# Sudaraka88/LDWeaver

Hardware: NVIDIA B200
Metric: weighted SNP-pair MI/sec (higher is better)
Workload: dtype int8 (tcgen05 kind::i8 with int32 accumulation of 28-bit fixed-point weights; fp32 MI epilogue, fp64 refinement of long-range links)

## Files before the change

### ldweaver_b200/csrc/mi_kernel.cuh

```cuda
#pragma once
#include "mi_types.h"
#include "umma.cuh"

namespace ldw {

constexpr int MI_EXP_WARPS = 6;
constexpr int MI_EXP_THREADS = 32 * MI_EXP_WARPS;
constexpr int MI_EPI_WARP0 = 8;
constexpr int MI_EPI_GROUPS = 4;
constexpr int MI_EPI_WARPS = 4 * MI_EPI_GROUPS;
constexpr int MI_EPI_THREADS = 32 * MI_EPI_WARPS;
constexpr int MI_THREADS = 32 * (MI_EPI_WARP0 + MI_EPI_WARPS);
#define LDW_STR2(x) #x
#define LDW_STR(x) LDW_STR2(x)
#define MI_REGS_CTRL 48
#define MI_REGS_EPI 96
static_assert(MI_EPI_WARP0 * 32 * MI_REGS_CTRL + MI_EPI_THREADS * MI_REGS_EPI <= MI_THREADS * ((65536 / MI_THREADS) & ~7), "register budget");
constexpr int MI_MAX_STAGES = 4;
constexpr uint32_t MI_ARR_BYTES = 128 * 128;
constexpr uint32_t MI_STAGE_REGION = 12 * MI_ARR_BYTES;
__host__ __device__ constexpr uint32_t mi_stage_need(int pa, int pb, int njlog2) {
  return (uint32_t)pa * MI_ARR_BYTES + 4u * (uint32_t)pb * (64u << njlog2);
}
__host__ __device__ constexpr int mi_stage_geo(int pa, int pb, int njlog2) {
  return mi_stage_need(pa, pb, njlog2) <= 3 * MI_ARR_BYTES ? 0 : mi_stage_need(pa, pb, njlog2) <= 4 * MI_ARR_BYTES ? 1 : 2;
}
__host__ __device__ constexpr int mi_geo_stages(int geo) { return 4 - geo; }
__host__ __device__ constexpr uint32_t mi_geo_bytes(int geo) { return geo == 0 ? 3 * MI_ARR_BYTES : geo == 1 ? 4 * MI_ARR_BYTES : 6 * MI_ARR_BYTES; }
constexpr uint32_t MI_JREC_BYTES = 128 * sizeof(Rec);
constexpr uint32_t MI_JDYN_BYTES = 128 * sizeof(ColDyn);
constexpr uint32_t MI_IREC_BYTES = 128 * sizeof(Rec);
constexpr uint32_t MI_IDYN_BYTES = 128 * sizeof(RowDyn);
constexpr uint32_t MI_BAR_BYTES = 512;
constexpr uint32_t MI_SMEM_BYTES = MI_STAGE_REGION + 2 * (MI_JREC_BYTES + MI_JDYN_BYTES) + MI_IREC_BYTES + MI_IDYN_BYTES + MI_BAR_BYTES + 1024;
static_assert(MI_SMEM_BYTES <= 232448, "shared memory budget (227 KB opt-in)");

__device__ __forceinline__ float lg2_fast(float x) {
  float y;
  asm("lg2.approx.ftz.f32 %0, %1;" : "=f"(y) : "f"(x));
  return y;
}
__device__ __forceinline__ uint32_t ld_volatile_u32(const uint32_t* p) {
  uint32_t v;
  asm volatile("ld.volatile.global.u32 %0, [%1];" : "=r"(v) : "l"(p));
  return v;
}

__host__ __device__ constexpr int mi_jc(int pa, int pb) {
  return (pa + 1) * (pb + 1) <= 4 ? 8 : (pa + 1) * (pb + 1) <= 9 ? 4 : (pa + 1) * (pb + 1) <= 12 ? 2 : 1;
}
__host__ __device__ constexpr int mi_njlog2(int pa, int pb) {
  return pa * pb == 1 ? 7 : pa * pb == 2 ? 6 : pa * pb <= 4 ? 5 : 4;
}

__device__ __noinline__ void lr_raise_threshold(const ScanParams& p, int lane) {
  constexpr int PER = MI_HIST_BINS / 32;
  uint32_t s = 0;
  for (int k = 0; k < PER; k++) s += ld_volatile_u32(p.hist + lane * PER + k);
  uint32_t suf = s;
#pragma unroll
  for (int o = 1; o < 32; o <<= 1) {
    uint32_t v = __shfl_down_sync(0xffffffffu, suf, o);
    if (lane + o < 32) suf += v;
  }
  unsigned m = __ballot_sync(0xffffffffu, suf >= p.kprime);
  if (m == 0) return;
  int sel = 31 - __clz(m);
  if (lane == sel) {
    uint32_t run = suf - s;
    for (int k = PER - 1; k >= 0; k--) {
      run += ld_volatile_u32(p.hist + lane * PER + k);
      if (run >= p.kprime) {
        atomicMax(p.tcand_bits, (uint32_t)(lane * PER + k) << 19);
        break;
      }
    }
  }
}

template <bool DBG>
__device__ __forceinline__ void timed_wait(uint64_t* bar, uint32_t parity, int tag, long long& acc) {
  if constexpr (DBG) {
    long long c0 = clock64();
    mbar_wait(bar, parity, tag);
    acc += clock64() - c0;
  } else {
    mbar_wait(bar, parity, tag);
  }
}

struct EpiCtx {
  int q, cg, lane, rank;
  uint32_t tflags;
// ... 267 lines not shown
  k.M = p.M;
  k.nf = p.nf; k.nt = p.nt;
  k.mul_a = 1u << p.sa; k.sb = p.sb;
  k.ragged = p.ragged != 0; k.dense = p.dense != 0;
  k.do_lr = !p.sr_only && !p.dense;
  k.has_sr = (c.tflags & TILE_HAS_SR) != 0;
  k.sr_out = p.sr_out;
  k.tcand = (k.do_lr && !p.emit_all) ? __uint_as_float(ld_volatile_u32(p.tcand_bits)) : -3.0e38f;
  uint32_t r0, r1;
  {
    const uint32_t rv = c.irec_saddr + (uint32_t)row * (uint32_t)sizeof(Rec);
    const uint4 v0 = lds128(rv), v1 = lds128(rv + (QC ? 32 : 16));
    uint4 v3 = make_uint4(0, 0, 0, 0);
    if (RA == 5) v3 = lds128(rv + 48);
    asm volatile("ld.shared.v2.u32 {%0, %1}, [%2];" : "=r"(r0), "=r"(r1) : "r"(c.idyn_saddr + (uint32_t)row * (uint32_t)sizeof(RowDyn)));
    {
      const uint32_t dep = (v0.x ^ v0.y ^ v0.z ^ v0.w ^ v1.x ^ v1.y ^ v1.z ^ v1.w ^ v3.x ^ v3.y ^ v3.z ^ r0 ^ r1);
      asm volatile("st.volatile.shared.u32 [%0], %1;" ::"r"(c.scr_saddr), "r"(dep) : "memory");
      __syncwarp();
      if (c.lane == 0) asm volatile("mbarrier.arrive.shared::cta.b64 _, [%0];" ::"r"(c.rempty_saddr) : "memory");
    }
    const uint32_t tt[5] = {v0.x, v0.y, v0.z, v0.w, v3.x}, tr[5] = {v1.x, v1.y, v1.z, v1.w, QC ? v3.z : v3.y};
    const float rf = QC ? p.rp_qc[RA - 2][RB - 2] : p.rp_plain[RA - 2][RB - 2];
#pragma unroll
    for (int a = 0; a < RA; a++) {
      k.Ti[a] = tt[a];
      k.rpad[a] = __uint_as_float(tr[a]) * rf;
    }
  }
  k.il = (int)r0;
  k.rtlq = __uint_as_float(r1) * k.qod;
// ... 47 lines not shown
  Rec* irec = reinterpret_cast<Rec*>(smem + MI_STAGE_REGION + 2 * (MI_JREC_BYTES + MI_JDYN_BYTES));
  RowDyn* idyn = reinterpret_cast<RowDyn*>(smem + MI_STAGE_REGION + 2 * (MI_JREC_BYTES + MI_JDYN_BYTES) + MI_IREC_BYTES);
  uint64_t* bars = reinterpret_cast<uint64_t*>(smem + MI_STAGE_REGION + 2 * (MI_JREC_BYTES + MI_JDYN_BYTES) + MI_IREC_BYTES + MI_IDYN_BYTES);
  uint64_t* full = bars;
  uint64_t* empty = bars + 4;
  uint64_t* ready = bars + 8;
  uint64_t* tfull = bars + 12;
  uint64_t* tempty = bars + 14;
  uint64_t* jfull = bars + 16;
  uint64_t* jempty = bars + 18;
  uint64_t* drained = bars + 20;
  uint64_t* rfull = bars + 21;
  uint64_t* rempty = bars + 22;
  uint32_t* tmem_slot = reinterpret_cast<uint32_t*>(bars + 23);
  uint32_t* thdr = reinterpret_cast<uint32_t*>(bars + 24);

  const int warp = threadIdx.x >> 5, lane = threadIdx.x & 31;
  const uint32_t rank = cluster_ctarank();
  if (warp == 0 && lane == 0) {
    tma_prefetch_desc(&tm.a);
    for (int i = 0; i < MI_MAX_STAGES; i++) {
      mbar_init(&full[i], 1); mbar_init(&empty[i], 1); mbar_init(&ready[i], 2 * MI_EXP_WARPS);
    }
    mbar_init(drained, 1);
    mbar_init(rfull, 1); mbar_init(rempty, MI_EPI_WARPS);
    for (int i = 0; i < 2; i++) {
      mbar_init(&tfull[i], 1); mbar_init(&tempty[i], 2 * MI_EPI_WARPS);
      mbar_init(&jfull[i], 1); mbar_init(&jempty[i], MI_EPI_WARPS);
    }
    fence_barrier_init();
  }
  if (warp == 2) tmem_alloc_pair(tmem_slot, 512);
  tc_fence_before();
  cluster_sync_all();
  tc_fence_after();
  const uint32_t tmem_base = *tmem_slot;
  const int tile0 = (int)(blockIdx.x >> 1), tstep = (int)(gridDim.x >> 1);

  if (warp < MI_EPI_WARP0) {
  asm volatile("setmaxnreg.dec.sync.aligned.u32 " LDW_STR(MI_REGS_CTRL) ";");
  if (warp == 0) {
    int st = 0; uint32_t phb = 0; int geo = -1; uint32_t dph = 0;
    int it = 0, rit = 0;
    long long w_jempty = 0, w_empty = 0, t_begin = DBG ? clock64() : 0;
    for (int t = tile0; t < p.n_tiles; t += tstep, it++) {
      const TileDesc td = p.tiles[t];
      const int PA = td.PA, PB = td.PB, NJ = 1 << td.njlog2, NJh = NJ >> 1;
      const int njidx = 7 - td.njlog2;
      const int g = mi_stage_geo(PA, PB, td.njlog2);
      const int nst = mi_geo_stages(g);
      const uint32_t sbytes = mi_geo_bytes(g);
      if (g != geo) {
        if (geo >= 0) { mbar_wait(drained, dph, 12); dph ^= 1; }
        geo = g; st = 0;
      }
      {
        const uint32_t stage_tx = (uint32_t)PA * MI_ARR_BYTES + (uint32_t)(PB * NJh * 128);
        const int a_row = td.a_row0 + (int)rank * 128, b_row = td.b_row0 + (int)rank * NJh;
        for (int kb = 0; kb < p.nkb; kb++) {
          timed_wait<DBG>(&empty[st], ((phb >> st) & 1) ^ 1, 11, w_empty);
          if (elect_one()) {
            uint8_t* sb = stage_base + st * sbytes;
            mbar_arrive_expect_tx(&full[st], stage_tx);
            for (int a = 0; a < PA; a++)
              tma_load_2d(sb + a * MI_ARR_BYTES, &tm.a, &full[st], kb * 128, a_row + a * td.a_pstride);
            uint8_t* sbB = sb + PA * MI_ARR_BYTES;
            for (int b = 0; b < PB; b++)
              tma_load_2d(sbB + b * NJh * 128, &tm.b[njidx], &full[st], kb * 128, b_row + b * td.b_pstride);
          }
          __syncwarp();
          phb ^= 1u << st;
          if (++st == nst) st = 0;
        }
      }
      const int jb = it & 1;
      timed_wait<DBG>(&jempty[jb], ((it >> 1) & 1) ^ 1, 10, w_jempty);
      if (elect_one()) {
        thdr[jb] = (uint32_t)PA | ((uint32_t)PB << 8) | ((uint32_t)td.njlog2 << 16) | ((uint32_t)(rank ? td.flags1 : td.flags) << 24);
        mbar_arrive_expect_tx(&jfull[jb], (uint32_t)NJ * (uint32_t)(sizeof(Rec) + sizeof(ColDyn)));
        bulk_load_1d(jrec + jb * 128, p.rec + (int64_t)(PA + 1 - 2) * p.rec_vstride + td.j_slot0, NJ * sizeof(Rec), &jfull[jb]);
        bulk_load_1d(jdyn + jb * 128, p.coldyn + td.j_dyn0, NJ * sizeof(ColDyn), &jfull[jb]);
      }
      __syncwarp();
      if (!((rank ? td.flags1 : td.flags) & TILE_NULL)) {
        timed_wait<DBG>(rempty, (uint32_t)(rit & 1) ^ 1, 13, w_jempty);
        if (elect_one()) {
          mbar_arrive_expect_tx(rfull, MI_IREC_BYTES + MI_IDYN_BYTES);
          bulk_load_1d(irec, p.rec + (int64_t)(PB + 1 - 2) * p.rec_vstride + td.i_slot0 + (int)rank * 128, MI_IREC_BYTES, rfull);
          bulk_load_1d(idyn, p.rowdyn + td.i_dyn0 + (int)rank * 128, MI_IDYN_BYTES, rfull);
        }
        __syncwarp();
        rit++;
      }
    }
    if (DBG && p.dbg && lane == 0) {
      p.dbg[blockIdx.x * 16 + 0] = (unsigned long long)(clock64() - t_begin);
      p.dbg[blockIdx.x * 16 + 1] = (unsigned long long)w_jempty;
      p.dbg[blockIdx.x * 16 + 2] = (unsigned long long)w_empty;
    }
  } else if (warp == 1) {
    if (rank == 0) {
    int st = 0; uint32_t phb = 0; int geo = -1; int as = 0; uint32_t aph = 0;
    long long w_tempty = 0, w_ready = 0, t_begin = DBG ? clock64() : 0;
    const uint32_t desc_hi = (uint32_t)(make_smem_desc_sw128(0) >> 32);
    for (int t = tile0; t < p.n_tiles; t += tstep) {
      const TileDesc td = p.tiles[t];
      const int PA = td.PA, PB = td.PB, NJ = 1 << td.njlog2;
      const int g = mi_stage_geo(PA, PB, td.njlog2);
      const int nst = mi_geo_stages(g);
      const uint32_t sbytes = mi_geo_bytes(g);
      if (g != geo) { geo = g; st = 0; }
      bool sw = false;
      if (t + tstep < p.n_tiles) {
        const TileDesc tn = p.tiles[t + tstep];
        sw = mi_stage_geo(tn.PA, tn.PB, tn.njlog2) != g;
      }
      const bool big = 2 * PA * PB * NJ > 256;
      const uint32_t ncols = (uint32_t)(2 * PB * NJ);
      const uint32_t idesc_u = make_idesc_u8(256, ncols);
      const uint32_t idesc_s = make_idesc_s8u8(256, ncols);
      uint32_t dbase;
      if (big) {
        for (int s2 = 0; s2 < 2; s2++) {
          timed_wait<DBG>(&tempty[as], aph ^ 1, 20, w_tempty);
          if (++as == 2) { as = 0; aph ^= 1; }
        }
        dbase = tmem_base;
      } else {
        timed_wait<DBG>(&tempty[as], aph ^ 1, 21, w_tempty);
        dbase = tmem_base + as * 256;
      }
      tc_fence_after();
      {
        const uint32_t boff = (uint32_t)PA * MI_ARR_BYTES;
        const uint32_t b2off = boff + (uint32_t)(PB * NJ * 128);
        for (int kb = 0; kb < p.nkb; kb++) {
          timed_wait<DBG>(&ready[st], (phb >> st) & 1, 22, w_ready);
          tc_fence_after();
          const uint32_t lo = ((smem_u32(stage_base + st * sbytes) & 0x3FFFFu) >> 4) | (1u << 16);
          if (elect_one()) {
            const uint64_t dBa = ((uint64_t)desc_hi << 32) | (lo + (boff >> 4));
            const uint64_t dBb = ((uint64_t)desc_hi << 32) | (lo + (b2off >> 4));
            const uint32_t acc0 = kb > 0 ? 1u : 0u;
            for (int a = 0; a < PA; a++) {
              const uint64_t dx = ((uint64_t)desc_hi << 32) | (lo + (uint32_t)((a * MI_ARR_BYTES) >> 4));
              const uint32_t dHL = dbase + (uint32_t)(a * 2 * PB * NJ);
              umma_i8_pair(dHL, dx, dBa, idesc_u, acc0);
              umma_i8_pair(dHL, dx, dBb, idesc_s, 1u);
#pragma unroll
              for (int kk = 1; kk < 4; kk++) {
                umma_i8_pair(dHL, dx + 2 * kk, dBa + 2 * kk, idesc_u, 1u);
                umma_i8_pair(dHL, dx + 2 * kk, dBb + 2 * kk, idesc_s, 1u);
              }
            }
            umma_commit_pair(&empty[st]);
          }
          __syncwarp();
          phb ^= 1u << st;
          if (++st == nst) st = 0;
        }
      }
      if (elect_one()) {
        if (sw) umma_commit_pair(drained);
        if (big) {
          umma_commit_pair(&tfull[0]);
          umma_commit_pair(&tfull[1]);
        } else {
          umma_commit_pair(&tfull[as]);
        }
      }
      __syncwarp();
      if (!big) {
        if (++as == 2) { as = 0; aph ^= 1; }
      }
    }
    if (DBG && p.dbg && lane == 0) {
      p.dbg[blockIdx.x * 16 + 3] = (unsigned long long)(clock64() - t_begin);
      p.dbg[blockIdx.x * 16 + 4] = (unsigned long long)w_tempty;
      p.dbg[blockIdx.x * 16 + 5] = (unsigned long long)w_ready;
    }
    }
  } else {
    const int h = (warp - 2) * 32 + lane;
    int st = 0; uint32_t phb = 0; int geo = -1;
    long long w_full = 0, t_begin = DBG ? clock64() : 0;
    for (int t = tile0; t < p.n_tiles; t += tstep) {
      const TileDesc td = p.tiles[t];
      const int PA = td.PA, PB = td.PB, NJh = (1 << td.njlog2) >> 1;
      const int brows = PB * NJh;
      const int g = mi_stage_geo(PA, PB, td.njlog2);
      const int nst = mi_geo_stages(g);
      const uint32_t sbytes = mi_geo_bytes(g);
      if (g != geo) { geo = g; st = 0; }
      for (int kb = 0; kb < p.nkb; kb++) {
        const int cl = h & 7;
        const uint8_t* dg = p.dig + (int64_t)kb * 128 + cl * 16;
        const uint4 g0 = __ldg(reinterpret_cast<const uint4*>(dg));
        const uint4 g1 = __ldg(reinterpret_cast<const uint4*>(dg + p.kpad));
        const uint4 g2 = __ldg(reinterpret_cast<const uint4*>(dg + 2 * p.kpad));
        const uint4 g3 = __ldg(reinterpret_cast<const uint4*>(dg + 3 * p.kpad));
        timed_wait<DBG>(&full[st], (phb >> st) & 1, 40, w_full);
        const uint32_t yb = smem_u32(stage_base + st * sbytes) + (uint32_t)PA * MI_ARR_BYTES;
        const uint32_t slot = (uint32_t)brows * 128u;
        for (int r = h >> 3; r < brows; r += MI_EXP_THREADS / 8) {
          const uint32_t addr = yb + (uint32_t)r * 128u + (uint32_t)((cl ^ (r & 7)) * 16);
          const uint4 y = lds128(addr);
          sts128(addr + slot, make_uint4(y.x & g1.x, y.y & g1.y, y.z & g1.z, y.w & g1.w));
          sts128(addr + 2 * slot, make_uint4(y.x & g2.x, y.y & g2.y, y.z & g2.z, y.w & g2.w));
          sts128(addr + 3 * slot, make_uint4(y.x & g3.x, y.y & g3.y, y.z & g3.z, y.w & g3.w));
          sts128(addr, make_uint4(y.x & g0.x, y.y & g0.y, y.z & g0.z, y.w & g0.w));
        }
        fence_proxy_async_smem();
        __syncwarp();
        if (lane == 0) mbar_arrive_cluster(&ready[st], 0);
        phb ^= 1u << st;
        if (++st == nst) st = 0;
      }
    }
    if (DBG && p.dbg && h == 0) {
      p.dbg[blockIdx.x * 16 + 12] = (unsigned long long)(clock64() - t_begin);
      p.dbg[blockIdx.x * 16 + 13] = (unsigned long long)w_full;
    }
  }
  } else {
    asm volatile("setmaxnreg.inc.sync.aligned.u32 " LDW_STR(MI_REGS_EPI) ";");
    EpiCtx c;
    c.q = warp & 3;
    c.cg = (warp - MI_EPI_WARP0) >> 2;
    c.lane = lane;
    c.rank = (int)rank;
    int as = 0; uint32_t aph = 0;
    int it = 0, rit = 0;
    long long w_jfull = 0, w_tfull = 0, t_begin = DBG ? clock64() : 0;
    c.irec_saddr = smem_u32(irec);
    c.idyn_saddr = smem_u32(idyn);
    c.rempty_saddr = smem_u32(rempty);
    c.scr_saddr = smem_u32(bars + 32) + (uint32_t)(warp - MI_EPI_WARP0) * 4u;
    for (int t = tile0; t < p.n_tiles; t += tstep, it++) {
      const int jb = it & 1;
      timed_wait<DBG>(&jfull[jb], (it >> 1) & 1, 30, w_jfull);
      uint32_t hdr;
      asm volatile("ld.shared.u32 %0, [%1];" : "=r"(hdr) : "r"(smem_u32(&thdr[jb])));
      const int tPA = (int)(hdr & 0xFF), tPB = (int)((hdr >> 8) & 0xFF);
      c.tflags = hdr >> 24;
      const int NJ = 1 << ((hdr >> 16) & 0xFF);
      const bool big = 2 * tPA * tPB * NJ > 256;
      if (!(c.tflags & TILE_NULL)) { timed_wait<DBG>(rfull, (uint32_t)(rit & 1), 34, w_jfull); rit++; }
      long long c1 = DBG ? clock64() : 0;
      c.jrec_saddr = smem_u32(jrec + jb * 128);
      c.jdyn_saddr = smem_u32(jdyn + jb * 128);
      if (big) {
        uint32_t ph0 = aph;
        mbar_wait(&tfull[as], ph0, 31);
        int as1 = as ^ 1;
        uint32_t ph1 = (as == 1) ? (aph ^ 1) : aph;
        mbar_wait(&tfull[as1], ph1, 32);
        c.tmem_base = tmem_base + ((uint32_t)(c.q * 32) << 16);
      } else {
        mbar_wait(&tfull[as], aph, 33);
        c.tmem_base = tmem_base + ((uint32_t)(c.q * 32) << 16) + as * 256;
      }
      if constexpr (DBG) w_tfull += clock64() - c1;
// ... 40 lines not shown
```

### ldweaver_b200/csrc/mi_scan.cu

```cuda
#include <algorithm>
#include <chrono>
#include <cmath>
#include <cub/cub.cuh>
#include <vector>

#include "../../include/ldw.h"
#include "ctx.h"
#include "hdw.h"
#include "mi_aux.cuh"
#include "mi_kernel.cuh"
#include "mi_scan.h"

using namespace ldw;

namespace {

struct Group {
  int32_t slot0 = 0, nslots = 0, row0 = 0, count = 0;
};

struct DevLinks {
  DevBuf pos1, pos2, c1, c2, len, blk, mi;
  int ensure(int64_t m) {
    size_t b4 = (size_t)(m > 0 ? m : 1) * 4, b8 = (size_t)(m > 0 ? m : 1) * 8;
    LDW_TRY(pos1.ensure(b4)); LDW_TRY(pos2.ensure(b4)); LDW_TRY(c1.ensure(b4)); LDW_TRY(c2.ensure(b4));
    LDW_TRY(len.ensure(b4)); LDW_TRY(blk.ensure(b4)); LDW_TRY(mi.ensure(b8));
    return 0;
  }
};

struct BlockDev {
  DevBuf rowdyn, coldyn, colinfo, tiles, from_idx, to_idx, rfl, rtl;
  PinnedBuf stage;
  cudaEvent_t uploaded = nullptr;
  cudaEvent_t done = nullptr, done2 = nullptr;
  bool used = false, used2 = false;
};

struct BlockHost {
  std::vector<RowDyn> rowdyn;
  std::vector<ColDyn> coldyn;
  std::vector<ColInfo> colinfo;
  std::vector<TileDesc> tiles;
  std::vector<int32_t> from_idx, to_idx;
  std::vector<uint8_t> rfl, rtl;
  int32_t nf = 0, nt = 0;
  int32_t n_real_tiles = 0;
  int diag = 0, ragged = 0;
  int64_t n_pairs = 0, n_sr = 0, n_lr = 0;
};

}

struct ScanWS {
  static constexpr int RING = 4;
  BlockDev ring[RING];
  BlockHost hring[RING];
  DevBuf d_dbg;
  struct LrBuf {
    DevBuf cand, vcand, mi64, state , hist;
    cudaEvent_t scan_done = nullptr, sel_done = nullptr;
    bool used = false, chain_valid = false;
// ... 497 lines not shown
    std::stable_sort(ord, ord + 16, [&](int a, int b) { return geo(a) != geo(b) ? geo(a) > geo(b) : cnt[a] < cnt[b]; });
    size_t off = 0;
    for (int k = 0; k < 16; k++) { beg[ord[k]] = off; off += cnt[ord[k]]; }
    std::vector<TileDesc> sorted(H.tiles.size());
    for (const TileDesc& t : H.tiles) sorted[beg[(t.PA - 1) * 4 + (t.PB - 1)]++] = t;
    H.tiles.swap(sorted);
  }
  H.n_real_tiles = (int32_t)H.tiles.size();
  if (!cfg.dense && H.n_real_tiles >= 1024) {
    const int np = 64;
    for (int k = 0; k < np; k++) H.tiles.push_back(H.tiles[(size_t)((2 * k + 1) * (int64_t)H.n_real_tiles / (2 * np))]);
  }
  return 0;
}

int upload_block(cudaStream_t st, BlockDev& D, const BlockHost& H) {
  struct Part { DevBuf* d; const void* src; size_t bytes; };
  Part parts[8] = {{&D.rowdyn, H.rowdyn.data(), H.rowdyn.size() * sizeof(RowDyn)},
                   {&D.coldyn, H.coldyn.data(), H.coldyn.size() * sizeof(ColDyn)},
                   {&D.colinfo, H.colinfo.data(), H.colinfo.size() * sizeof(ColInfo)},
                   {&D.tiles, H.tiles.data(), H.tiles.size() * sizeof(TileDesc)},
                   {&D.from_idx, H.from_idx.data(), H.from_idx.size() * 4},
                   {&D.to_idx, H.to_idx.data(), H.to_idx.size() * 4},
                   {&D.rfl, H.rfl.data(), H.rfl.size()},
                   {&D.rtl, H.rtl.data(), H.rtl.size()}};
  size_t total = 0;
  for (auto& p : parts) total += (p.bytes + 255) & ~(size_t)255;
  LDW_TRY(D.stage.ensure(total + 256));
  size_t off = 0;
  for (auto& p : parts) {
    LDW_TRY(p.d->ensure(std::max<size_t>(p.bytes, 16)));
    if (p.bytes) {
      memcpy(D.stage.as<uint8_t>() + off, p.src, p.bytes);
      LDW_CUDA(cudaMemcpyAsync(p.d->p, D.stage.as<uint8_t>() + off, p.bytes, cudaMemcpyHostToDevice, st));
    }
    off += (p.bytes + 255) & ~(size_t)255;
  }
  return 0;
}

void fill_scan_params(const ldw_mi_plan* P, const BlockDev& D, const BlockHost& H, const ScanCfg& cfg, ScanParams& sp) {
  memset(&sp, 0, sizeof(sp));
  sp.tiles = D.tiles.as<TileDesc>();
  sp.n_tiles = H.n_real_tiles;
  sp.rec = P->d_rec.as<Rec>();
  sp.rec_vstride = P->nslots;
  sp.rowdyn = D.rowdyn.as<RowDyn>();
  sp.coldyn = D.coldyn.as<ColDyn>();
  sp.nkb = (int32_t)(P->Kpad / 128);
  sp.nf = H.nf; sp.nt = H.nt;
  sp.diag = H.diag; sp.ragged = H.ragged;
  sp.qcorr = (!H.diag && !(cfg.flags & LDW_SCAN_IDEAL_Q)) ? 1 : 0;
  sp.sr_only = (cfg.flags & LDW_SCAN_SR_ONLY) ? 1 : 0;
  sp.dig = P->d_dig.as<uint8_t>();
  sp.kpad = P->Kpad;
  sp.rfl_arr = D.rfl.as<uint8_t>();
  sp.rtl_arr = D.rtl.as<uint8_t>();
  sp.sa = P->sa;
  sp.sb = P->sb;
// ... 2 lines not shown
  for (int a = 0; a < 4; a++)
    for (int b = 0; b < 4; b++) {
      double ri = a + 2, rj = b + 2;
      double den = P->neff + 0.5 * ri * rj;
      const float den_f = (float)den, rkT = 1.0f / sp.kT, rden = 1.0f / den_f;
      sp.scale[a][b] = (float)(M_LN2 / den) * sp.kT;
      sp.q0s[a][b] = (float)(0.25 * ri * rj / den) * rkT;
      sp.qod[a][b] = (float)(0.25 / den) * rkT;
      sp.rp_qc[a][b] = rden * rkT;
      sp.rp_plain[a][b] = den_f * sp.kT;
    }
}

int launch_scan(const ldw_mi_plan* P, const ScanParams& sp, cudaStream_t st, int reserve = 0) {
  if (sp.n_tiles <= 0) return 0;
  int grid = 2 * std::min<int>(sp.n_tiles, std::max(1, (P->ctx->num_sms - reserve) / 2));
  if (sp.dbg) mi_scan_kernel<true><<<grid, MI_THREADS, MI_SMEM_BYTES, st>>>(P->tm, sp);
  else mi_scan_kernel<false><<<grid, MI_THREADS, MI_SMEM_BYTES, st>>>(P->tm, sp);
  LDW_CUDA(cudaGetLastError());
  return 0;
}

RefineParams make_refine_params(const ldw_mi_plan* P, const BlockDev& D, const BlockHost& H, const ScanCfg& cfg) {
  RefineParams R;
  R.codes = P->codes_dev;
  R.S = P->S;
  R.w = P->d_w.as<double>();
  R.p64 = P->d_p64.as<double>();
  R.r = P->d_r.as<uint8_t>();
  R.mask = P->d_mask.as<uint8_t>();
  R.from_idx = D.from_idx.as<int32_t>();
// ... 85 lines not shown
      for (int j = i; j < P->nranges; j++) {
        if (k == 0) { bf = i; bt = j; found = true; break; }
        k--;
      }
    if (!found) return set_error(LDW_ERR_ARG, "block index out of range");
  }
  ScanCfg cfg{1e15, 0.0, 0, 0, 0};
  cfg.dense = 1;
  BlockHost& H = W->hring[0];
  BlockDev& D = W->ring[0];
  int e = prepare_block(P, bf, bt, cfg, H);
  if (e > 1) return e;
  if (nf_out) *nf_out = H.nf;
  if (nt_out) *nt_out = H.nt;
  if (!mi_out) return 0;
  LDW_TRY(upload_block(st, D, H));
  size_t cells = (size_t)H.nf * H.nt;
  LDW_TRY(W->d_dense.ensure(cells * 4));
  LDW_CUDA(cudaMemsetAsync(W->d_dense.p, 0, cells * 4, st));
  ScanParams sp;
  fill_scan_params(P, D, H, cfg, sp);
  sp.dense = 1;
  sp.dense_out = W->d_dense.as<float>();
  LDW_TRY(launch_scan(P, sp, st));
  DevBuf d64;
  LDW_TRY(d64.alloc(cells * 8));
  f32_to_f64_kernel<<<(unsigned)((cells + 255) / 256), 256, 0, st>>>(W->d_dense.as<float>(), (int64_t)cells, d64.as<double>());
  LDW_CUDA(cudaMemcpyAsync(mi_out, d64.p, cells * 8, cudaMemcpyDeviceToHost, st));
  LDW_CUDA(cudaStreamSynchronize(st));
  return 0;
// ... 263 lines not shown
    if (D.used2) { LDW_CUDA(cudaEventSynchronize(D.done2)); D.used2 = false; }
    ScanWS::LrBuf& L = W->lr[seq % ScanWS::NLR];
    uint32_t* d_count = L.state.as<uint32_t>();
    uint32_t* d_tcand = d_count + 1;
    uint32_t* d_overflow = d_count + 2;
    uint32_t* d_chain = d_chain2;
    auto hp0 = std::chrono::steady_clock::now();
    int e;
    if (seq == 0 && first_guess == (int64_t)b && first_rc >= 0 && first_rc <= 1 && !force_emit_all && !cap_override) {
      e = first_rc;
      first_rc = -1;
    } else {
      e = prepare_block(P, blocks[b].bf, blocks[b].bt, cfg, H);
    }
    if (e > 1) return e;
    LDW_TRY(upload_block(P->ctx->upload_stream, D, H));
    LDW_CUDA(cudaEventRecord(D.uploaded, P->ctx->upload_stream));
    LDW_CUDA(cudaStreamWaitEvent(st, D.uploaded, 0));
    host_prep_ms += std::chrono::duration<double, std::milli>(std::chrono::steady_clock::now() - hp0).count();
    D.used = true;
    ScanParams sp;
    fill_scan_params(P, D, H, cfg, sp);
    sp.sr_out = W->d_sr_f32.as<float>() + s.sr_base;
    if (dbg_block >= 0 && (int64_t)b == dbg_block) {
      LDW_TRY(W->d_dbg.ensure(4096 * 16 * 8));
      LDW_CUDA(cudaMemsetAsync(W->d_dbg.p, 0, 4096 * 16 * 8, st));
      sp.dbg = W->d_dbg.as<unsigned long long>();
    }
    const bool lr = !sr_only && s.n_lr > 0;
    const int emit_all = force_emit_all || s.emit_all;
    uint32_t cap = cap_override ? cap_override : s.cap;
    if (lr) {
      if (L.used) LDW_CUDA(cudaStreamWaitEvent(st, L.sel_done, 0));
      const int n_pilot = (int)H.tiles.size() - H.n_real_tiles;
      if (seq == 0 && use_chain && !emit_all && n_pilot > 0) {
        mi_block_begin_kernel<<<1, 256, 0, st>>>(d_count, L.hist.as<uint32_t>(), d_chain, 0);
        ScanParams pp = sp;
        pp.tiles = D.tiles.as<TileDesc>() + H.n_real_tiles;
        pp.n_tiles = n_pilot;
        pp.cand = L.cand.as<Cand>(); pp.cand_cap = cap; pp.cand_count = d_count; pp.tcand_bits = d_tcand;
        pp.hist = L.hist.as<uint32_t>(); pp.kprime = s.kprime; pp.delta = s.delta ? s.delta : 1; pp.overflow = d_overflow;
        pp.emit_all = 1;
        pp.dbg = nullptr;
        LDW_TRY(launch_scan(P, pp, st, 0));
        mi_pilot_seed_kernel<<<1, 1024, 0, st>>>(L.cand.as<Cand>(), d_count, cap, (unsigned long long)s.k_lo, (double)s.n_lr, d_chain);
        LDW_CUDA(cudaGetLastError());
        n_launches += 3;
      }
      if (force_seed >= 0.f && use_chain && !emit_all) {
        static_assert(sizeof(float) == 4, "float bits");
        LDW_CUDA(cudaMemcpyAsync(d_chain, &force_seed, 4, cudaMemcpyHostToDevice, st));
        LDW_CUDA(cudaStreamSynchronize(st));
      }
      mi_block_begin_kernel<<<1, 256, 0, st>>>(d_count, L.hist.as<uint32_t>(), d_chain, (use_chain && !emit_all) ? 1 : 0);
// ... 304 lines not shown
    {
      double em = 0;
      for (size_t b = 0; b < blocks.size(); b++)
        if (!sel[b].skip && sel[b].n_lr > 0 && !sr_only) em = std::max(em, (double)P->results[b].eps_obs);
      stats_out->eps_obs_max = em;
    }
  }
  if (dbg_block >= 0 && W->d_dbg.p) {
    std::vector<unsigned long long> h(4096 * 16);
    cudaMemcpy(h.data(), W->d_dbg.p, h.size() * 8, cudaMemcpyDeviceToHost);
    double s[16] = {0};
    int nb = 0;
    for (int c = 0; c < 4096; c++)
      if (h[c * 16 + 3]) { nb++; for (int k = 0; k < 16; k++) s[k] += (double)h[c * 16 + k]; }
    if (nb) {
      fprintf(stderr, "ldw dbg block %lld (%d CTAs, kilo-cycles avg): producer total %.0f wait_jempty %.0f wait_empty %.0f | "
              "mma total %.0f wait_tempty %.0f wait_ready %.0f | expander total %.0f wait_full %.0f | epi(first) total %.0f "
              "wait_jfull %.0f wait_tfull %.0f | epi(last) total %.0f wait_jfull %.0f wait_tfull %.0f\n", (long long)dbg_block, nb,
              s[0] / nb / 1e3, s[1] / nb / 1e3, s[2] / nb / 1e3, s[3] / nb / 1e3, s[4] / nb / 1e3, s[5] / nb / 1e3, s[12] / nb / 1e3,
              s[13] / nb / 1e3, s[6] / nb / 1e3, s[7] / nb / 1e3, s[8] / nb / 1e3, s[9] / nb / 1e3, s[10] / nb / 1e3, s[11] / nb / 1e3);
    }
  }
  kev_cleanup();
  cudaEventDestroy(ev0); cudaEventDestroy(ev1); cudaEventDestroy(ev2); cudaEventDestroy(ev3);
  lap("borderline + stats (host)");
  return 0;
}
```

### ldweaver_b200/csrc/mi_types.h

```cpp
#pragma once
#include <cuda.h>
#include <stdint.h>

namespace ldw {

struct __align__(16) Rec {
  uint32_t T[4];
  float rp[4];
  float q[4];
  uint32_t T4;
  float rp4;
  float q4;
  uint32_t pad;
};
static_assert(sizeof(Rec) == 64, "Rec must be 64 bytes");

struct RowDyn {
  int32_t il;
  float rtl;
};

struct __align__(16) ColDyn {
  int32_t jl;
  float rfl;
  int32_t a0, a1, b0, b1;
  uint32_t baseU, baseL;
};
static_assert(sizeof(ColDyn) == 32, "ColDyn must be 32 bytes");

enum : uint32_t { TILE_HAS_SR = 1u, TILE_NULL = 2u };

struct __align__(16) TileDesc {
  int32_t a_row0, a_pstride;
  int32_t b_row0, b_pstride;
  int32_t i_slot0, j_slot0;
  int32_t i_dyn0, j_dyn0;
  uint8_t PA, PB, njlog2, flags;
  uint8_t flags1, pad8[3];
  int32_t pad[2];
};
static_assert(sizeof(TileDesc) == 48, "TileDesc must be 48 bytes");

struct Cand {
  int32_t il, jl;
  float mi;
};

constexpr int MI_HIST_BINS = 4096;

struct ScanParams {
  const TileDesc* tiles;
  int32_t n_tiles;
  const Rec* rec;
  int64_t rec_vstride;
  const RowDyn* rowdyn;
  const ColDyn* coldyn;
  int32_t nkb;
  int32_t nf, nt;
  int32_t diag, ragged, qcorr, sr_only, dense, emit_all;
  const uint8_t* rfl_arr;
  const uint8_t* rtl_arr;
  float kT;
  uint32_t sa, sb;
  uint32_t M;
  float scale[4][4];
  float q0s[4][4];
  float qod[4][4];
// ... 23 lines not shown
```

Baseline: 85.61 billion.

## Keep A-operand rows resident in shared memory across consecutive tiles sharing a row block

Adds a resident geometry for small PA/nkb tiles. The A-operand k-blocks for a row block are loaded once into shared memory with their own full/empty barriers and reused across consecutive tiles with the same a_row0; only B is streamed through the stage ring. The static strided tile assignment is replaced by a host-built per-CTA-pair linked walk of contiguous chunks, so same-row tiles land on the same CTA pair. Row records are loaded once per run rather than per tile. This cuts repeated A TMA traffic and row-record reloads, but leaves fewer B stages (possibly two) and adds host walk construction and extra barrier bookkeeping.

Result: slower. 73.65 billion, median of 6 (-14.0%).

```diff
diff --git a/ldweaver_b200/csrc/mi_kernel.cuh b/ldweaver_b200/csrc/mi_kernel.cuh
--- a/ldweaver_b200/csrc/mi_kernel.cuh
+++ b/ldweaver_b200/csrc/mi_kernel.cuh
@@ -17,6 +17,7 @@
 #define MI_REGS_EPI 96
 static_assert(MI_EPI_WARP0 * 32 * MI_REGS_CTRL + MI_EPI_THREADS * MI_REGS_EPI <= MI_THREADS * ((65536 / MI_THREADS) & ~7), "register budget");
 constexpr int MI_MAX_STAGES = 4;
+constexpr int MI_RES_MAX_NKB = 5;
 constexpr uint32_t MI_ARR_BYTES = 128 * 128;
 constexpr uint32_t MI_STAGE_REGION = 12 * MI_ARR_BYTES;
 __host__ __device__ constexpr uint32_t mi_stage_need(int pa, int pb, int njlog2) {
@@ -25,8 +26,34 @@
 __host__ __device__ constexpr int mi_stage_geo(int pa, int pb, int njlog2) {
   return mi_stage_need(pa, pb, njlog2) <= 3 * MI_ARR_BYTES ? 0 : mi_stage_need(pa, pb, njlog2) <= 4 * MI_ARR_BYTES ? 1 : 2;
 }
-__host__ __device__ constexpr int mi_geo_stages(int geo) { return 4 - geo; }
-__host__ __device__ constexpr uint32_t mi_geo_bytes(int geo) { return geo == 0 ? 3 * MI_ARR_BYTES : geo == 1 ? 4 * MI_ARR_BYTES : 6 * MI_ARR_BYTES; }
+__host__ __device__ constexpr int mi_njlog2(int pa, int pb) {
+  return pa * pb == 1 ? 7 : pa * pb == 2 ? 6 : pa * pb <= 4 ? 5 : 4;
+}
+constexpr int MI_GEO_RES = 3;
+constexpr uint32_t MI_HDR_LAST = 1u << 30;
+constexpr int MI_APH_BIT = 8;
+__host__ __device__ constexpr uint32_t mi_res_abytes(int pa, int nkb) { return (uint32_t)pa * (uint32_t)nkb * MI_ARR_BYTES; }
+__host__ __device__ constexpr uint32_t mi_res_sbytes(int pb, int njlog2) { return 4u * (uint32_t)pb * (64u << njlog2); }
+__host__ __device__ constexpr int mi_tile_geo(int pa, int pb, int njlog2, int nkb) {
+  return nkb <= MI_RES_MAX_NKB && mi_res_abytes(pa, nkb) + 2 * mi_res_sbytes(pb, njlog2) <= MI_STAGE_REGION
+             ? MI_GEO_RES + (pa - 1) * 4 + (pb - 1)
+             : mi_stage_geo(pa, pb, njlog2);
+}
+__host__ __device__ constexpr int mi_geo_pa(int geo) { return (geo - MI_GEO_RES) / 4 + 1; }
+__host__ __device__ constexpr int mi_geo_pb(int geo) { return (geo - MI_GEO_RES) % 4 + 1; }
+__host__ __device__ constexpr uint32_t mi_geo_bytes(int geo) {
+  return geo == 0 ? 3 * MI_ARR_BYTES : geo == 1 ? 4 * MI_ARR_BYTES : geo == 2 ? 6 * MI_ARR_BYTES
+                                                                : mi_res_sbytes(mi_geo_pb(geo), mi_njlog2(mi_geo_pa(geo), mi_geo_pb(geo)));
+}
+__host__ __device__ constexpr uint32_t mi_geo_abytes(int geo, int nkb) { return geo < MI_GEO_RES ? 0u : mi_res_abytes(mi_geo_pa(geo), nkb); }
+__host__ __device__ constexpr int mi_geo_stages(int geo, int nkb) {
+  return geo < MI_GEO_RES ? 4 - geo
+                          : (int)((MI_STAGE_REGION - mi_geo_abytes(geo, nkb)) / mi_geo_bytes(geo)) < MI_MAX_STAGES
+                                ? (int)((MI_STAGE_REGION - mi_geo_abytes(geo, nkb)) / mi_geo_bytes(geo))
+                                : MI_MAX_STAGES;
+}
+static_assert(mi_tile_geo(2, 2, 5, 5) >= MI_GEO_RES && mi_geo_stages(mi_tile_geo(2, 2, 5, 5), 5) == 2, "(2, 2) at 640 sequences: 160 KB of rows + two 16 KB stages");
+static_assert(mi_tile_geo(3, 1, 5, 5) < MI_GEO_RES && mi_tile_geo(1, 1, 7, 6) < MI_GEO_RES, "PA >= 3 and nkb > 5 stream");
 constexpr uint32_t MI_JREC_BYTES = 128 * sizeof(Rec);
 constexpr uint32_t MI_JDYN_BYTES = 128 * sizeof(ColDyn);
 constexpr uint32_t MI_IREC_BYTES = 128 * sizeof(Rec);
@@ -48,9 +75,6 @@
 
 __host__ __device__ constexpr int mi_jc(int pa, int pb) {
   return (pa + 1) * (pb + 1) <= 4 ? 8 : (pa + 1) * (pb + 1) <= 9 ? 4 : (pa + 1) * (pb + 1) <= 12 ? 2 : 1;
-}
-__host__ __device__ constexpr int mi_njlog2(int pa, int pb) {
-  return pa * pb == 1 ? 7 : pa * pb == 2 ? 6 : pa * pb <= 4 ? 5 : 4;
 }
 
 __device__ __noinline__ void lr_raise_threshold(const ScanParams& p, int lane) {
@@ -77,6 +101,8 @@
     }
   }
 }
+
+__device__ __forceinline__ int mi_walk_first(const ScanParams& p, int pair) { return pair < p.n_chunks ? p.chunk_beg[pair] : -1; }
 
 template <bool DBG>
 __device__ __forceinline__ void timed_wait(uint64_t* bar, uint32_t parity, int tag, long long& acc) {
@@ -374,7 +400,7 @@
     uint4 v3 = make_uint4(0, 0, 0, 0);
     if (RA == 5) v3 = lds128(rv + 48);
     asm volatile("ld.shared.v2.u32 {%0, %1}, [%2];" : "=r"(r0), "=r"(r1) : "r"(c.idyn_saddr + (uint32_t)row * (uint32_t)sizeof(RowDyn)));
-    {
+    if (c.tflags & TILE_RLAST) {
       const uint32_t dep = (v0.x ^ v0.y ^ v0.z ^ v0.w ^ v1.x ^ v1.y ^ v1.z ^ v1.w ^ v3.x ^ v3.y ^ v3.z ^ r0 ^ r1);
       asm volatile("st.volatile.shared.u32 [%0], %1;" ::"r"(c.scr_saddr), "r"(dep) : "memory");
       __syncwarp();
@@ -452,6 +478,9 @@
   uint64_t* rempty = bars + 22;
   uint32_t* tmem_slot = reinterpret_cast<uint32_t*>(bars + 23);
   uint32_t* thdr = reinterpret_cast<uint32_t*>(bars + 24);
+  uint64_t* afull = bars + 40;
+  uint64_t* aempty = bars + 45;
+  static_assert(8 * (45 + MI_RES_MAX_NKB) <= MI_BAR_BYTES, "barrier area");
 
   const int warp = threadIdx.x >> 5, lane = threadIdx.x & 31;
   const uint32_t rank = cluster_ctarank();
@@ -461,6 +490,7 @@
       mbar_init(&full[i], 1); mbar_init(&empty[i], 1); mbar_init(&ready[i], 2 * MI_EXP_WARPS);
     }
     mbar_init(drained, 1);
+    for (int i = 0; i < MI_RES_MAX_NKB; i++) { mbar_init(&afull[i], 1); mbar_init(&aempty[i], 1); }
     mbar_init(rfull, 1); mbar_init(rempty, MI_EPI_WARPS);
     for (int i = 0; i < 2; i++) {
       mbar_init(&tfull[i], 1); mbar_init(&tempty[i], 2 * MI_EPI_WARPS);
@@ -473,36 +503,51 @@
   cluster_sync_all();
   tc_fence_after();
   const uint32_t tmem_base = *tmem_slot;
-  const int tile0 = (int)(blockIdx.x >> 1), tstep = (int)(gridDim.x >> 1);
+  const int tile0 = mi_walk_first(p, (int)(blockIdx.x >> 1));
 
   if (warp < MI_EPI_WARP0) {
   asm volatile("setmaxnreg.dec.sync.aligned.u32 " LDW_STR(MI_REGS_CTRL) ";");
   if (warp == 0) {
     int st = 0; uint32_t phb = 0; int geo = -1; uint32_t dph = 0;
     int it = 0, rit = 0;
-    long long w_jempty = 0, w_empty = 0, t_begin = DBG ? clock64() : 0;
-    for (int t = tile0; t < p.n_tiles; t += tstep, it++) {
+    long long w_jempty = 0, w_empty = 0, w_aempty = 0, t_begin = DBG ? clock64() : 0;
+    for (int t = tile0; t >= 0; t = p.tiles[t].next, it++) {
       const TileDesc td = p.tiles[t];
       const int PA = td.PA, PB = td.PB, NJ = 1 << td.njlog2, NJh = NJ >> 1;
       const int njidx = 7 - td.njlog2;
-      const int g = mi_stage_geo(PA, PB, td.njlog2);
-      const int nst = mi_geo_stages(g);
+      const uint32_t myfl = rank ? td.flags1 : td.flags;
+      const int g = mi_tile_geo(PA, PB, td.njlog2, p.nkb);
+      const int nst = mi_geo_stages(g, p.nkb);
       const uint32_t sbytes = mi_geo_bytes(g);
+      const bool res = g >= MI_GEO_RES;
+      const bool arel = res && (myfl & TILE_AREL);
+      const uint32_t boff = res ? mi_geo_abytes(g, p.nkb) : (uint32_t)PA * MI_ARR_BYTES;
       if (g != geo) {
         if (geo >= 0) { mbar_wait(drained, dph, 12); dph ^= 1; }
         geo = g; st = 0;
       }
       {
-        const uint32_t stage_tx = (uint32_t)PA * MI_ARR_BYTES + (uint32_t)(PB * NJh * 128);
+        const uint32_t stage_tx = (res ? 0u : (uint32_t)PA * MI_ARR_BYTES) + (uint32_t)(PB * NJh * 128);
         const int a_row = td.a_row0 + (int)rank * 128, b_row = td.b_row0 + (int)rank * NJh;
         for (int kb = 0; kb < p.nkb; kb++) {
+          if (arel) {
+            timed_wait<DBG>(&aempty[kb], ((phb >> MI_APH_BIT) & 1) ^ 1, 14, w_aempty);
+            if (elect_one()) {
+              uint8_t* sa = stage_base + kb * PA * MI_ARR_BYTES;
+              mbar_arrive_expect_tx(&afull[kb], (uint32_t)PA * MI_ARR_BYTES);
+              for (int a = 0; a < PA; a++)
+                tma_load_2d(sa + a * MI_ARR_BYTES, &tm.a, &afull[kb], kb * 128, a_row + a * td.a_pstride);
+            }
+            __syncwarp();
+          }
           timed_wait<DBG>(&empty[st], ((phb >> st) & 1) ^ 1, 11, w_empty);
           if (elect_one()) {
             uint8_t* sb = stage_base + st * sbytes;
             mbar_arrive_expect_tx(&full[st], stage_tx);
-            for (int a = 0; a < PA; a++)
-              tma_load_2d(sb + a * MI_ARR_BYTES, &tm.a, &full[st], kb * 128, a_row + a * td.a_pstride);
-            uint8_t* sbB = sb + PA * MI_ARR_BYTES;
+            if (!res)
+              for (int a = 0; a < PA; a++)
+                tma_load_2d(sb + a * MI_ARR_BYTES, &tm.a, &full[st], kb * 128, a_row + a * td.a_pstride);
+            uint8_t* sbB = sb + boff;
             for (int b = 0; b < PB; b++)
               tma_load_2d(sbB + b * NJh * 128, &tm.b[njidx], &full[st], kb * 128, b_row + b * td.b_pstride);
           }
@@ -510,17 +555,18 @@
           phb ^= 1u << st;
           if (++st == nst) st = 0;
         }
+        if (arel) phb ^= 1u << MI_APH_BIT;
       }
       const int jb = it & 1;
       timed_wait<DBG>(&jempty[jb], ((it >> 1) & 1) ^ 1, 10, w_jempty);
       if (elect_one()) {
-        thdr[jb] = (uint32_t)PA | ((uint32_t)PB << 8) | ((uint32_t)td.njlog2 << 16) | ((uint32_t)(rank ? td.flags1 : td.flags) << 24);
+        thdr[jb] = (uint32_t)PA | ((uint32_t)PB << 8) | ((uint32_t)td.njlog2 << 16) | (myfl << 24) | (td.next < 0 ? MI_HDR_LAST : 0u);
         mbar_arrive_expect_tx(&jfull[jb], (uint32_t)NJ * (uint32_t)(sizeof(Rec) + sizeof(ColDyn)));
         bulk_load_1d(jrec + jb * 128, p.rec + (int64_t)(PA + 1 - 2) * p.rec_vstride + td.j_slot0, NJ * sizeof(Rec), &jfull[jb]);
         bulk_load_1d(jdyn + jb * 128, p.coldyn + td.j_dyn0, NJ * sizeof(ColDyn), &jfull[jb]);
       }
       __syncwarp();
-      if (!((rank ? td.flags1 : td.flags) & TILE_NULL)) {
+      if (myfl & TILE_RLOAD) {
         timed_wait<DBG>(rempty, (uint32_t)(rit & 1) ^ 1, 13, w_jempty);
         if (elect_one()) {
           mbar_arrive_expect_tx(rfull, MI_IREC_BYTES + MI_IDYN_BYTES);
@@ -535,23 +581,26 @@
       p.dbg[blockIdx.x * 16 + 0] = (unsigned long long)(clock64() - t_begin);
       p.dbg[blockIdx.x * 16 + 1] = (unsigned long long)w_jempty;
       p.dbg[blockIdx.x * 16 + 2] = (unsigned long long)w_empty;
+      p.dbg[blockIdx.x * 16 + 14] = (unsigned long long)w_aempty;
     }
   } else if (warp == 1) {
     if (rank == 0) {
     int st = 0; uint32_t phb = 0; int geo = -1; int as = 0; uint32_t aph = 0;
     long long w_tempty = 0, w_ready = 0, t_begin = DBG ? clock64() : 0;
     const uint32_t desc_hi = (uint32_t)(make_smem_desc_sw128(0) >> 32);
-    for (int t = tile0; t < p.n_tiles; t += tstep) {
+    for (int t = tile0; t >= 0; t = p.tiles[t].next) {
       const TileDesc td = p.tiles[t];
       const int PA = td.PA, PB = td.PB, NJ = 1 << td.njlog2;
-      const int g = mi_stage_geo(PA, PB, td.njlog2);
-      const int nst = mi_geo_stages(g);
+      const int g = mi_tile_geo(PA, PB, td.njlog2, p.nkb);
+      const int nst = mi_geo_stages(g, p.nkb);
       const uint32_t sbytes = mi_geo_bytes(g);
+      const bool res = g >= MI_GEO_RES;
+      const bool alast = res && (td.flags & TILE_ALAST);
       if (g != geo) { geo = g; st = 0; }
       bool sw = false;
-      if (t + tstep < p.n_tiles) {
-        const TileDesc tn = p.tiles[t + tstep];
-        sw = mi_stage_geo(tn.PA, tn.PB, tn.njlog2) != g;
+      if (td.next >= 0) {
+        const TileDesc tn = p.tiles[td.next];
+        sw = mi_tile_geo(tn.PA, tn.PB, tn.njlog2, p.nkb) != g;
       }
       const bool big = 2 * PA * PB * NJ > 256;
       const uint32_t ncols = (uint32_t)(2 * PB * NJ);
@@ -570,18 +619,19 @@
       }
       tc_fence_after();
       {
-        const uint32_t boff = (uint32_t)PA * MI_ARR_BYTES;
+        const uint32_t boff = res ? mi_geo_abytes(g, p.nkb) : (uint32_t)PA * MI_ARR_BYTES;
         const uint32_t b2off = boff + (uint32_t)(PB * NJ * 128);
         for (int kb = 0; kb < p.nkb; kb++) {
           timed_wait<DBG>(&ready[st], (phb >> st) & 1, 22, w_ready);
           tc_fence_after();
           const uint32_t lo = ((smem_u32(stage_base + st * sbytes) & 0x3FFFFu) >> 4) | (1u << 16);
+          const uint32_t alo = res ? ((smem_u32(stage_base + kb * PA * MI_ARR_BYTES) & 0x3FFFFu) >> 4) | (1u << 16) : lo;
           if (elect_one()) {
             const uint64_t dBa = ((uint64_t)desc_hi << 32) | (lo + (boff >> 4));
             const uint64_t dBb = ((uint64_t)desc_hi << 32) | (lo + (b2off >> 4));
             const uint32_t acc0 = kb > 0 ? 1u : 0u;
             for (int a = 0; a < PA; a++) {
-              const uint64_t dx = ((uint64_t)desc_hi << 32) | (lo + (uint32_t)((a * MI_ARR_BYTES) >> 4));
+              const uint64_t dx = ((uint64_t)desc_hi << 32) | (alo + (uint32_t)((a * MI_ARR_BYTES) >> 4));
               const uint32_t dHL = dbase + (uint32_t)(a * 2 * PB * NJ);
               umma_i8_pair(dHL, dx, dBa, idesc_u, acc0);
               umma_i8_pair(dHL, dx, dBb, idesc_s, 1u);
@@ -592,6 +642,7 @@
               }
             }
             umma_commit_pair(&empty[st]);
+            if (alast) umma_commit_pair(&aempty[kb]);
           }
           __syncwarp();
           phb ^= 1u << st;
@@ -621,14 +672,17 @@
   } else {
     const int h = (warp - 2) * 32 + lane;
     int st = 0; uint32_t phb = 0; int geo = -1;
-    long long w_full = 0, t_begin = DBG ? clock64() : 0;
-    for (int t = tile0; t < p.n_tiles; t += tstep) {
+    long long w_full = 0, w_afull = 0, t_begin = DBG ? clock64() : 0;
+    for (int t = tile0; t >= 0; t = p.tiles[t].next) {
       const TileDesc td = p.tiles[t];
       const int PA = td.PA, PB = td.PB, NJh = (1 << td.njlog2) >> 1;
       const int brows = PB * NJh;
-      const int g = mi_stage_geo(PA, PB, td.njlog2);
-      const int nst = mi_geo_stages(g);
+      const int g = mi_tile_geo(PA, PB, td.njlog2, p.nkb);
+      const int nst = mi_geo_stages(g, p.nkb);
       const uint32_t sbytes = mi_geo_bytes(g);
+      const bool res = g >= MI_GEO_RES;
+      const bool arel = res && (td.flags & TILE_AREL);
+      const uint32_t yb0 = smem_u32(stage_base) + (res ? mi_geo_abytes(g, p.nkb) : (uint32_t)PA * MI_ARR_BYTES);
       if (g != geo) { geo = g; st = 0; }
       for (int kb = 0; kb < p.nkb; kb++) {
         const int cl = h & 7;
@@ -638,7 +692,7 @@
         const uint4 g2 = __ldg(reinterpret_cast<const uint4*>(dg + 2 * p.kpad));
         const uint4 g3 = __ldg(reinterpret_cast<const uint4*>(dg + 3 * p.kpad));
         timed_wait<DBG>(&full[st], (phb >> st) & 1, 40, w_full);
-        const uint32_t yb = smem_u32(stage_base + st * sbytes) + (uint32_t)PA * MI_ARR_BYTES;
+        const uint32_t yb = yb0 + st * sbytes;
         const uint32_t slot = (uint32_t)brows * 128u;
         for (int r = h >> 3; r < brows; r += MI_EXP_THREADS / 8) {
           const uint32_t addr = yb + (uint32_t)r * 128u + (uint32_t)((cl ^ (r & 7)) * 16);
@@ -649,15 +703,18 @@
           sts128(addr, make_uint4(y.x & g0.x, y.y & g0.y, y.z & g0.z, y.w & g0.w));
         }
         fence_proxy_async_smem();
+        if (arel) timed_wait<DBG>(&afull[kb], (phb >> MI_APH_BIT) & 1, 41, w_afull);
         __syncwarp();
         if (lane == 0) mbar_arrive_cluster(&ready[st], 0);
         phb ^= 1u << st;
         if (++st == nst) st = 0;
       }
+      if (arel) phb ^= 1u << MI_APH_BIT;
     }
     if (DBG && p.dbg && h == 0) {
       p.dbg[blockIdx.x * 16 + 12] = (unsigned long long)(clock64() - t_begin);
       p.dbg[blockIdx.x * 16 + 13] = (unsigned long long)w_full;
+      p.dbg[blockIdx.x * 16 + 15] = (unsigned long long)w_afull;
     }
   }
   } else {
@@ -674,16 +731,17 @@
     c.idyn_saddr = smem_u32(idyn);
     c.rempty_saddr = smem_u32(rempty);
     c.scr_saddr = smem_u32(bars + 32) + (uint32_t)(warp - MI_EPI_WARP0) * 4u;
-    for (int t = tile0; t < p.n_tiles; t += tstep, it++) {
+    for (bool more = tile0 >= 0; more; it++) {
       const int jb = it & 1;
       timed_wait<DBG>(&jfull[jb], (it >> 1) & 1, 30, w_jfull);
       uint32_t hdr;
       asm volatile("ld.shared.u32 %0, [%1];" : "=r"(hdr) : "r"(smem_u32(&thdr[jb])));
+      more = !(hdr & MI_HDR_LAST);
       const int tPA = (int)(hdr & 0xFF), tPB = (int)((hdr >> 8) & 0xFF);
       c.tflags = hdr >> 24;
       const int NJ = 1 << ((hdr >> 16) & 0xFF);
       const bool big = 2 * tPA * tPB * NJ > 256;
-      if (!(c.tflags & TILE_NULL)) { timed_wait<DBG>(rfull, (uint32_t)(rit & 1), 34, w_jfull); rit++; }
+      if (c.tflags & TILE_RLOAD) { timed_wait<DBG>(rfull, (uint32_t)(rit & 1), 34, w_jfull); rit++; }
       long long c1 = DBG ? clock64() : 0;
       c.jrec_saddr = smem_u32(jrec + jb * 128);
       c.jdyn_saddr = smem_u32(jdyn + jb * 128);
diff --git a/ldweaver_b200/csrc/mi_scan.cu b/ldweaver_b200/csrc/mi_scan.cu
--- a/ldweaver_b200/csrc/mi_scan.cu
+++ b/ldweaver_b200/csrc/mi_scan.cu
@@ -30,7 +30,7 @@
 };
 
 struct BlockDev {
-  DevBuf rowdyn, coldyn, colinfo, tiles, from_idx, to_idx, rfl, rtl;
+  DevBuf rowdyn, coldyn, colinfo, tiles, chunks, from_idx, to_idx, rfl, rtl;
   PinnedBuf stage;
   cudaEvent_t uploaded = nullptr;
   cudaEvent_t done = nullptr, done2 = nullptr;
@@ -46,6 +46,8 @@
   std::vector<uint8_t> rfl, rtl;
   int32_t nf = 0, nt = 0;
   int32_t n_real_tiles = 0;
+  std::vector<int32_t> chunks;
+  int32_t n_real_chunks = 0, walk_pairs = 0;
   int diag = 0, ragged = 0;
   int64_t n_pairs = 0, n_sr = 0, n_lr = 0;
 };
@@ -573,12 +575,70 @@
   return 0;
 }
 
+#ifndef MI_RUN_TILES
+#define MI_RUN_TILES 16
+#endif
+
+int scan_pairs(const ldw_mi_plan* P, int reserve) { return std::max(1, (P->ctx->num_sms - reserve) / 2); }
+
+void build_walk(const ldw_mi_plan* P, BlockHost& H, int npairs) {
+  const int nkb = (int)(P->Kpad / 128);
+  const int32_t n = H.n_real_tiles;
+  H.chunks.clear();
+  for (int32_t k0 = 0, k1; k0 < n; k0 = k1) {
+    const TileDesc& t0 = H.tiles[k0];
+    for (k1 = k0 + 1; k1 < n && H.tiles[k1].PA == t0.PA && H.tiles[k1].PB == t0.PB; k1++) {}
+    const int64_t len = k1 - k0;
+    const int64_t L = mi_tile_geo(t0.PA, t0.PB, t0.njlog2, nkb) >= MI_GEO_RES ? MI_RUN_TILES : 1;
+    const int64_t full = len / (L * npairs) * (L * npairs), rest = len - full;
+    for (int64_t o = 0; o < full; o += L) H.chunks.push_back(k0 + (int32_t)o);
+    for (int64_t i = 0, o = full; i < npairs && o < len; i++) {
+      H.chunks.push_back(k0 + (int32_t)o);
+      o += rest / npairs + (i < rest % npairs ? 1 : 0);
+    }
+  }
+  H.n_real_chunks = (int32_t)H.chunks.size();
+  H.chunks.push_back(n);
+  H.walk_pairs = npairs;
+  constexpr uint8_t WALK = TILE_AREL | TILE_ALAST | TILE_RLOAD | TILE_RLAST;
+  auto set_flags = [](TileDesc* t, int32_t m) {
+    for (int32_t i = 0; i < m; i++) {
+      t[i].flags &= ~WALK; t[i].flags1 &= ~WALK;
+      if (i == 0) { t[i].flags |= TILE_AREL; t[i].flags1 |= TILE_AREL; }
+      if (i == m - 1) { t[i].flags |= TILE_ALAST; t[i].flags1 |= TILE_ALAST; }
+    }
+    for (int h = 0; h < 2; h++) {
+      int32_t first = -1, last = -1;
+      for (int32_t i = 0; i < m; i++)
+        if (!((h ? t[i].flags1 : t[i].flags) & TILE_NULL)) { if (first < 0) first = i; last = i; }
+      if (first < 0) continue;
+      (h ? t[first].flags1 : t[first].flags) |= TILE_RLOAD;
+      (h ? t[last].flags1 : t[last].flags) |= TILE_RLAST;
+    }
+  };
+  for (int32_t c = 0; c < H.n_real_chunks; c++) {
+    for (int32_t b = H.chunks[c], e; b < H.chunks[c + 1]; b = e) {
+      for (e = b + 1; e < H.chunks[c + 1] && H.tiles[e].a_row0 == H.tiles[b].a_row0; e++) {}
+      set_flags(&H.tiles[b], e - b);
+    }
+    for (int32_t t = H.chunks[c]; t < H.chunks[c + 1]; t++)
+      H.tiles[t].next = t + 1 < H.chunks[c + 1] ? t + 1 : c + npairs < H.n_real_chunks ? H.chunks[c + npairs] : -1;
+  }
+  const int32_t np = (int32_t)H.tiles.size() - n, pilot_pairs = scan_pairs(P, 0);
+  for (int32_t k = 0; k <= np; k++) H.chunks.push_back(k);
+  for (int32_t k = 0; k < np; k++) {
+    set_flags(&H.tiles[n + k], 1);
+    H.tiles[n + k].next = k + pilot_pairs < np ? k + pilot_pairs : -1;
+  }
+}
+
 int upload_block(cudaStream_t st, BlockDev& D, const BlockHost& H) {
   struct Part { DevBuf* d; const void* src; size_t bytes; };
-  Part parts[8] = {{&D.rowdyn, H.rowdyn.data(), H.rowdyn.size() * sizeof(RowDyn)},
+  Part parts[9] = {{&D.rowdyn, H.rowdyn.data(), H.rowdyn.size() * sizeof(RowDyn)},
                    {&D.coldyn, H.coldyn.data(), H.coldyn.size() * sizeof(ColDyn)},
                    {&D.colinfo, H.colinfo.data(), H.colinfo.size() * sizeof(ColInfo)},
                    {&D.tiles, H.tiles.data(), H.tiles.size() * sizeof(TileDesc)},
+                   {&D.chunks, H.chunks.data(), H.chunks.size() * sizeof(int32_t)},
                    {&D.from_idx, H.from_idx.data(), H.from_idx.size() * 4},
                    {&D.to_idx, H.to_idx.data(), H.to_idx.size() * 4},
                    {&D.rfl, H.rfl.data(), H.rfl.size()},
@@ -602,6 +662,9 @@
   memset(&sp, 0, sizeof(sp));
   sp.tiles = D.tiles.as<TileDesc>();
   sp.n_tiles = H.n_real_tiles;
+  sp.chunk_beg = D.chunks.as<int32_t>();
+  sp.n_chunks = H.n_real_chunks;
+  sp.walk_pairs = H.walk_pairs;
   sp.rec = P->d_rec.as<Rec>();
   sp.rec_vstride = P->nslots;
   sp.rowdyn = D.rowdyn.as<RowDyn>();
@@ -634,7 +697,9 @@
 
 int launch_scan(const ldw_mi_plan* P, const ScanParams& sp, cudaStream_t st, int reserve = 0) {
   if (sp.n_tiles <= 0) return 0;
-  int grid = 2 * std::min<int>(sp.n_tiles, std::max(1, (P->ctx->num_sms - reserve) / 2));
+  if (sp.walk_pairs != scan_pairs(P, reserve))
+    return set_error(LDW_ERR_INTERNAL, "scan: tile walk built for %d CTA pairs, launch has %d", sp.walk_pairs, scan_pairs(P, reserve));
+  int grid = 2 * std::min<int>(sp.n_chunks, scan_pairs(P, reserve));
   if (sp.dbg) mi_scan_kernel<true><<<grid, MI_THREADS, MI_SMEM_BYTES, st>>>(P->tm, sp);
   else mi_scan_kernel<false><<<grid, MI_THREADS, MI_SMEM_BYTES, st>>>(P->tm, sp);
   LDW_CUDA(cudaGetLastError());
@@ -750,6 +815,7 @@
   if (nf_out) *nf_out = H.nf;
   if (nt_out) *nt_out = H.nt;
   if (!mi_out) return 0;
+  build_walk(P, H, scan_pairs(P, 0));
   LDW_TRY(upload_block(st, D, H));
   size_t cells = (size_t)H.nf * H.nt;
   LDW_TRY(W->d_dense.ensure(cells * 4));
@@ -1043,6 +1109,8 @@
       e = prepare_block(P, blocks[b].bf, blocks[b].bt, cfg, H);
     }
     if (e > 1) return e;
+    const bool lr = !sr_only && s.n_lr > 0;
+    build_walk(P, H, scan_pairs(P, lr ? scan_reserve : 0));
     LDW_TRY(upload_block(P->ctx->upload_stream, D, H));
     LDW_CUDA(cudaEventRecord(D.uploaded, P->ctx->upload_stream));
     LDW_CUDA(cudaStreamWaitEvent(st, D.uploaded, 0));
@@ -1056,7 +1124,6 @@
       LDW_CUDA(cudaMemsetAsync(W->d_dbg.p, 0, 4096 * 16 * 8, st));
       sp.dbg = W->d_dbg.as<unsigned long long>();
     }
-    const bool lr = !sr_only && s.n_lr > 0;
     const int emit_all = force_emit_all || s.emit_all;
     uint32_t cap = cap_override ? cap_override : s.cap;
     if (lr) {
@@ -1067,6 +1134,9 @@
         ScanParams pp = sp;
         pp.tiles = D.tiles.as<TileDesc>() + H.n_real_tiles;
         pp.n_tiles = n_pilot;
+        pp.chunk_beg = D.chunks.as<int32_t>() + H.n_real_chunks + 1;
+        pp.n_chunks = n_pilot;
+        pp.walk_pairs = scan_pairs(P, 0);
         pp.cand = L.cand.as<Cand>(); pp.cand_cap = cap; pp.cand_count = d_count; pp.tcand_bits = d_tcand;
         pp.hist = L.hist.as<uint32_t>(); pp.kprime = s.kprime; pp.delta = s.delta ? s.delta : 1; pp.overflow = d_overflow;
         pp.emit_all = 1;
@@ -1401,11 +1471,12 @@
     for (int c = 0; c < 4096; c++)
       if (h[c * 16 + 3]) { nb++; for (int k = 0; k < 16; k++) s[k] += (double)h[c * 16 + k]; }
     if (nb) {
-      fprintf(stderr, "ldw dbg block %lld (%d CTAs, kilo-cycles avg): producer total %.0f wait_jempty %.0f wait_empty %.0f | "
-              "mma total %.0f wait_tempty %.0f wait_ready %.0f | expander total %.0f wait_full %.0f | epi(first) total %.0f "
-              "wait_jfull %.0f wait_tfull %.0f | epi(last) total %.0f wait_jfull %.0f wait_tfull %.0f\n", (long long)dbg_block, nb,
-              s[0] / nb / 1e3, s[1] / nb / 1e3, s[2] / nb / 1e3, s[3] / nb / 1e3, s[4] / nb / 1e3, s[5] / nb / 1e3, s[12] / nb / 1e3,
-              s[13] / nb / 1e3, s[6] / nb / 1e3, s[7] / nb / 1e3, s[8] / nb / 1e3, s[9] / nb / 1e3, s[10] / nb / 1e3, s[11] / nb / 1e3);
+      fprintf(stderr, "ldw dbg block %lld (%d CTAs, kilo-cycles avg): producer total %.0f wait_jempty %.0f wait_empty %.0f "
+              "wait_aempty %.0f | mma total %.0f wait_tempty %.0f wait_ready %.0f | expander total %.0f wait_full %.0f wait_afull %.0f | "
+              "epi(first) total %.0f wait_jfull %.0f wait_tfull %.0f | epi(last) total %.0f wait_jfull %.0f wait_tfull %.0f\n",
+              (long long)dbg_block, nb, s[0] / nb / 1e3, s[1] / nb / 1e3, s[2] / nb / 1e3, s[14] / nb / 1e3, s[3] / nb / 1e3,
+              s[4] / nb / 1e3, s[5] / nb / 1e3, s[12] / nb / 1e3, s[13] / nb / 1e3, s[15] / nb / 1e3, s[6] / nb / 1e3,
+              s[7] / nb / 1e3, s[8] / nb / 1e3, s[9] / nb / 1e3, s[10] / nb / 1e3, s[11] / nb / 1e3);
     }
   }
   kev_cleanup();
diff --git a/ldweaver_b200/csrc/mi_types.h b/ldweaver_b200/csrc/mi_types.h
--- a/ldweaver_b200/csrc/mi_types.h
+++ b/ldweaver_b200/csrc/mi_types.h
@@ -28,7 +28,7 @@
 };
 static_assert(sizeof(ColDyn) == 32, "ColDyn must be 32 bytes");
 
-enum : uint32_t { TILE_HAS_SR = 1u, TILE_NULL = 2u };
+enum : uint32_t { TILE_HAS_SR = 1u, TILE_NULL = 2u, TILE_AREL = 4u, TILE_ALAST = 8u, TILE_RLOAD = 16u, TILE_RLAST = 32u };
 
 struct __align__(16) TileDesc {
   int32_t a_row0, a_pstride;
@@ -37,7 +37,8 @@
   int32_t i_dyn0, j_dyn0;
   uint8_t PA, PB, njlog2, flags;
   uint8_t flags1, pad8[3];
-  int32_t pad[2];
+  int32_t next;
+  int32_t pad;
 };
 static_assert(sizeof(TileDesc) == 48, "TileDesc must be 48 bytes");
 
@@ -51,6 +52,8 @@
 struct ScanParams {
   const TileDesc* tiles;
   int32_t n_tiles;
+  const int32_t* chunk_beg;
+  int32_t n_chunks, walk_pairs;
   const Rec* rec;
   int64_t rec_vstride;
   const RowDyn* rowdyn;
```
